# vvvwo/KSS-ICP

Hardware: AMD Instinct MI355X
Metric: icp_iterations_per_sec (higher is better)
Workload: dtype f32; 1 GPU; C2: one 100000x100000 uniform-sphere pair per GPU, 50 fixed ICP iterations + fitness pass per step (exact NN + cov reduce + host 3x3 SVD), R_z(10deg), jitter 1e-3; n_src=100000, n_tgt=100000, pairs_per_gpu=1, nn_engine=cell list + brute-force fallback, nn_arithmetic=reference (no fma)

## Files before the change

### kss-icp_amd/csrc/kss_ctx.hpp

```cpp
#pragma once
#include <dlfcn.h>
#include <hip/hip_runtime.h>

#include <algorithm>
#include <atomic>
#include <chrono>
#include <cmath>
#include <cstdio>
#include <cstdlib>
#include <cstring>
#include <mutex>
#include <string>
#include <thread>
#include <vector>

#include "kss_internal.hpp"
#include "kss_host_pool.hpp"

using namespace kss;

struct DevBuf {
    void* p = nullptr;
    size_t cap = 0;
};

struct kss_ctx {
    int device = 0;
    int cu_count = 0;
    hipStream_t stream = nullptr;
    bool own_stream = false;
    std::string err;
    int nn_mode = KSS_NN_AUTO;
    double grid_stats[8] = {0, 0, 0, 0, 0, 0, 0, 0};
    double last_setup_ms = 0, last_loop_ms = 0;
    double t_launch_us = 0, t_wait_us = 0, t_host_us = 0;
    bool timing = false;
    bool tables_staged = false;
    int64_t stats_ns = -1, stats_nt = -1;

    DevBuf tgt4, src0, cur[2], keys, partials, sums, nn_work, red_work, pair_red, state, cs, scratch_a,
        scratch_b, scratch_c, stage_src, stage_tgt, stage_idx, stage_d2, stage_out, g_counts, g_start, g_cursor,
        g_bsums, g_sorted, g_list, g_count, g_bbox, g_partials, g_start2, g_pairs, g_stamps, g_pos, g_nnst, res_pos, res_wc, res_perm, cand_tags, pack_seg, reg_s, reg_t, reg_p, reg_all, reg_f, reg_g, oct_pts, oct_cen, oct_a, oct_b, oct_tmp, pair_ticket, pre_partials, pre_state, g_rowpair, g_gate;
    HostPool pool;
    std::vector<kss_ctx*> workers;
    std::vector<unsigned long long> last_stamps;
    int stamps_nblk = 0; unsigned long long stamps_seq = 0;
    std::vector<float> h_bbox;
    unsigned int* h_box = nullptr; unsigned int* h_box_dev = nullptr; size_t h_box_bytes = 0;
    unsigned box_tag = 0; int box_rows = 0;
    double evals_sum = 0.0, evals_launches = 0.0;
    void* h_sums = nullptr;  size_t h_sums_cap = 0;
    void* h_sums_dev = nullptr;
    unsigned long long* h_seq = nullptr;
    unsigned long long* h_seq_dev = nullptr;
    size_t h_seq_bytes = 0;
    struct Gated {
        int supported = -1;
        bool want_next = false;
        bool pending = false;
        bool chain = false;
        int steps_left = 0;
        int max_steps = 1;
        int slot = 0;
        unsigned long long seq = 0;
        int32_t stamp = 0;
        const void* d_in = nullptr; void* d_out = nullptr;
        bool fma = false, full = false, want_full = false; double max_d2 = 0.0;
    } gated;
    bool ws_dirty = false;
    bool defer_wait = false;
    PairState* h_xf = nullptr; PairState* h_xf_dev = nullptr;
    bool fit_last = false;
    bool nn_have = false;
    PairState* bar_state = nullptr; int bar_state_cap = 0; bool bar_state_failed = false;
    unsigned int* gate_bar = nullptr;
    unsigned int* res_gate = nullptr; int res_gate_cap = 0; bool res_gate_failed = false;
    unsigned res_launches = 0;
    double res_passes = 0.0;
    int cand_cap = 0, cand_cap_pad = -1, cand_cap_fma = -1;
    int spec_judge = -1; double spec_threshold = 0.0; bool spec_ran = false, spec_cancelled = false;
    std::chrono::steady_clock::time_point res_backoff[2] = {};
    unsigned long long seq = 0;
    void* h_state = nullptr; size_t h_state_cap = 0;

    int prof = 0;
    unsigned prof_tick[KSS_K_COUNT] = {};
    struct EvPair { hipEvent_t a, b; };
    std::vector<EvPair> ev[KSS_K_COUNT];
    std::vector<EvPair> ev_pool;
    double prof_ms[KSS_K_COUNT] = {0};
    int64_t prof_n[KSS_K_COUNT] = {0};
};

static inline int set_err(kss_ctx* c, int code, const char* what, hipError_t e = hipSuccess) {
    if (c) {
        c->err = what;
        if (e != hipSuccess) { c->err += ": "; c->err += hipGetErrorString(e); }
    }
    return code;
}

#define HIPCHK(ctx, call)                                                        \
    do {                                                                         \
        hipError_t e_ = (call);                                                  \
        if (e_ != hipSuccess) return set_err((ctx), KSS_ERR_HIP, #call, e_);     \
    } while (0)

static inline int ensure(kss_ctx* c, DevBuf& b, size_t bytes) {
    if (bytes <= b.cap) return KSS_OK;
    if (b.p) {
        HIPCHK(c, hipStreamSynchronize(c->stream));
        HIPCHK(c, hipFree(b.p));
        b.p = nullptr; b.cap = 0;
    }
    size_t want = bytes + bytes / 8 + 256;
    hipError_t e = hipMalloc(&b.p, want);
    if (e != hipSuccess) { b.p = nullptr; return set_err(c, KSS_ERR_NOMEM, "hipMalloc", e); }
    b.cap = want;
    return KSS_OK;
}

static inline int ensure_zeroed(kss_ctx* c, DevBuf& b, size_t bytes) {
    const size_t before = b.cap;
    const int rc = ensure(c, b, bytes);
    if (rc != KSS_OK) return rc;
    if (b.cap != before && hipMemsetAsync(b.p, 0, b.cap, c->stream) != hipSuccess) return set_err(c, KSS_ERR_HIP, "hipMemsetAsync(zero-at-rest buffer)");
    return KSS_OK;
}

static inline int ensure_pinned(kss_ctx* c, void*& p, size_t& cap, size_t bytes) {
    if (bytes <= cap) return KSS_OK;
    if (p) { HIPCHK(c, hipStreamSynchronize(c->stream)); HIPCHK(c, hipHostFree(p)); p = nullptr; cap = 0; }
    size_t want = bytes * 2 + 256;
    hipError_t e = hipHostMalloc(&p, want, hipHostMallocMapped);
    if (e != hipSuccess) { p = nullptr; return set_err(c, KSS_ERR_NOMEM, "hipHostMalloc", e); }
    cap = want;
    if (&p == &c->h_sums) {
        void* d = nullptr;
        HIPCHK(c, hipHostGetDevicePointer(&d, p, 0));
        c->h_sums_dev = d;
    }
    return KSS_OK;
}

#define KCHK(expr)                     \
    do {                               \
        int rc_ = (expr);              \
        if (rc_ != KSS_OK) return rc_; \
    } while (0)

// ... 54 lines not shown
```

### kss-icp_amd/csrc/kss_engine.hip

```cpp
#pragma clang fp contract(off)

#include <emmintrin.h>

#include "kss_ctx.hpp"

namespace kss {

static int restore_zero_at_rest(kss_ctx* c);
static bool resident_gate_available(kss_ctx* c, int npairs);

static int resident_rows_limit(kss_ctx* c) {
    if (c->cu_count <= 0) {
        hipDeviceProp_t prop;
        c->cu_count = hipGetDeviceProperties(&prop, c->device) == hipSuccess && prop.multiProcessorCount > 0 ? prop.multiProcessorCount : 1;
        (void)hipGetLastError();
    }
    return c->cu_count;
}

constexpr int PUB_PAIRS = 32;
static int ensure_pub(kss_ctx* c, int npairs = PUB_PAIRS);

struct PairGeom {
    int64_t ns, nt;
// ... 469 lines not shown
    }
    return true;
}

static int wait_pair(kss_ctx* c, int p, unsigned long long want) {
    for (long spin = 0; spin < 2000000; ++spin) {
        if (collect_pair(c, p, want)) return KSS_OK;
        __builtin_ia32_pause();
    }
    return KSS_ERR_HIP;
}

static int wait_seq(kss_ctx* c, int npairs = 1, unsigned long long want = 0, const int* active = nullptr, bool* not_published = nullptr) {
    if (!want) want = c->seq;
    bool slow = false;
    for (int p = npairs - 1; p >= 0; --p) {
        if (active && !active[p]) continue;
        if (!slow && wait_pair(c, p, want) == KSS_OK) continue;
        if (!slow) {
            gated_cancel(c);
            HIPCHK(c, hipStreamSynchronize(c->stream));
            slow = true;
        }
        if (!collect_pair(c, p, want)) {
            if (not_published) *not_published = true;
            return set_err(c, KSS_ERR_HIP, "kernel finished without publishing its result");
        }
    }
    return KSS_OK;
}

int ensure_pub_slots(kss_ctx* c) { return ensure_pub(c); }
int wait_slots(kss_ctx* c, int nslots, double* out) {
    const unsigned long long want = c->seq;
    auto collect = [&]() -> bool {
        for (int k = nslots - 1; k >= 0; --k) {
            unsigned long long bits;
            if (!slot_value(c->h_seq, k, want, &bits)) return false;
            std::memcpy(&out[k], &bits, sizeof(double));
        }
        return true;
    };
    for (long spin = 0; spin < 2000000; ++spin) {
        if (collect()) return KSS_OK;
        __builtin_ia32_pause();
    }
    HIPCHK(c, hipStreamSynchronize(c->stream));
    if (!collect()) return set_err(c, KSS_ERR_HIP, "kernel finished without publishing its result");
    return KSS_OK;
}

static bool gated_available(kss_ctx* c) {
    static const bool want = getenv("KSS_GATED") == nullptr || atoi(getenv("KSS_GATED")) != 0;
    if (!want || !c->own_stream || kss_live_contexts().load() != 1) return false;
    if (c->gated.supported < 0) {
        c->gated.supported = 0;
        static const bool want_bar = getenv("KSS_GATE_BAR") == nullptr || atoi(getenv("KSS_GATE_BAR")) != 0;
        hipDeviceProp_t prop;
        void* bar = nullptr;
        if (want_bar && hipGetDeviceProperties(&prop, c->device) == hipSuccess && prop.isLargeBar &&
            hipExtMallocWithFlags(&bar, 4096, hipDeviceMallocFinegrained) == hipSuccess && bar) {
            if (hipMemset(bar, 0, 4096) == hipSuccess && hipDeviceSynchronize() == hipSuccess) {
                c->gate_bar = (unsigned int*)bar;
                c->gated.supported = 1;
                return true;
            }
            hipFree(bar);
        }
        (void)hipGetLastError();
        void *x = nullptr, *xd = nullptr;
        if (ensure(c, c->g_gate, 256) == KSS_OK && hipMemsetAsync(c->g_gate.p, 0, 256, c->stream) == hipSuccess &&
            hipHostMalloc(&x, 2 * sizeof(PairState), hipHostMallocMapped) == hipSuccess && hipHostGetDevicePointer(&xd, x, 0) == hipSuccess) {
            std::memset(x, 0, 2 * sizeof(PairState));
            c->h_xf = (PairState*)x; c->h_xf_dev = (PairState*)xd;
            c->gated.supported = 1;
        } else {
            (void)hipGetLastError();
            if (x) hipHostFree(x);
        }
    }
    return c->gated.supported == 1;
}

static void gated_release(kss_ctx* c, const PairState& st, int skip) {
    if (c->gate_bar) {
        int words[16];
        std::memcpy(words, &st, sizeof st);
        words[14] = skip;
        unsigned int* slot = c->gate_bar + 32 * c->gated.slot;
        static const long torn_at = getenv("KSS_TEST_TORN_GATE") ? atol(getenv("KSS_TEST_TORN_GATE")) : -1;
        static long released = 0;
        const bool torn = ++released == torn_at;
        for (int pass = torn ? 0 : 1; pass < 2; ++pass) {
            for (int g = 0; g < 5; ++g) {
                const unsigned tag = (unsigned)c->gated.stamp + kss_mix3((unsigned)words[3 * g], (unsigned)words[3 * g + 1], (unsigned)words[3 * g + 2]);
                const int w1 = pass == 0 && g == 1 ? words[3 * g + 1] ^ 0x00010000 : words[3 * g + 1];
                const __m128i v = _mm_set_epi32((int)tag, words[3 * g + 2], w1, words[3 * g]);
                _mm_store_si128((__m128i*)(slot + 4 * g), v);
            }
            _mm_sfence();
            if (pass == 0) {
                const auto t0 = std::chrono::steady_clock::now();
                while (std::chrono::duration<double, std::micro>(std::chrono::steady_clock::now() - t0).count() < 200.0) __builtin_ia32_pause();
            }
        }
    } else {
        PairState* rec = &c->h_xf[c->gated.slot];
        for (int k = 0; k < 12; ++k) rec->m[k] = st.m[k];
        rec->active = st.active; rec->apply = st.apply; rec->pad[0] = skip;
        __atomic_store_n(&rec->pad[1], c->gated.stamp, __ATOMIC_RELEASE);
    }
    kss_ctx::Gated& G = c->gated;
    if (!skip && --G.steps_left > 0) {
        G.slot ^= 1;
        G.stamp += 1;
        G.seq += 1;
        const void* in = G.d_out; G.d_out = const_cast<void*>(G.d_in); G.d_in = in;
    } else {
        G.pending = false;
        G.steps_left = 0;
    }
}

static void gated_cancel(kss_ctx* c) {
    if (!c->gated.pending) return;
    PairState none;
    std::memset(&none, 0, sizeof none);
    gated_release(c, none, 1);
}

struct GatedGuard {
    kss_ctx* c;
    explicit GatedGuard(kss_ctx* c_) : c(c_) {}
    ~GatedGuard() { gated_cancel(c); c->gated.want_next = false; }
};

static PassArgs pass_args(kss_ctx* c, const IcpPlan& pl, const float4* d_in, float4* d_out, double max_d2,
                          int32_t* d_idx_out, float* d_d2_out) {
    PassArgs a;
    std::memset(&a, 0, sizeof a);
    a.src_in = d_in; a.src_out = d_out;
    a.cell_start = (const int32_t*)c->g_start.p + 1;
    a.sorted = (const float4*)c->g_sorted.p;
    a.tgt4 = (const float4*)c->tgt4.p;
    a.nn_win = (float4*)c->g_pos.p;
    a.nn_state = (float2*)c->g_nnst.p;
    static const float skin = getenv("KSS_SKIN") ? (float)atof(getenv("KSS_SKIN")) : 0.25f;
    a.skin = skin;
    a.chain_len = 1;
    static const int gate_polls = getenv("KSS_GATE_POLLS") ? atoi(getenv("KSS_GATE_POLLS")) : (1 << 22);
    a.gate_polls = gate_polls;
    a.chained = d_in != (const float4*)c->src0.p ? 1 : c->fit_last ? 2 : 0;
    a.src_last0 = (const float4*)c->cur[0].p; a.src_last1 = (const float4*)c->cur[1].p;
    a.keys = (unsigned long long*)c->keys.p;
    a.list = (int32_t*)c->g_list.p; a.list_count = (int32_t*)c->g_count.p;
    a.total_rows = pl.total_rows;
    static const bool noprev = getenv("KSS_GRID_NOPREV") != nullptr;
    a.use_prev = !noprev && c->nn_have ? 1 : 0;
    a.max_d2 = max_d2;
    a.rows = (double*)c->partials.p; a.tickets = (int32_t*)c->pair_ticket.p;
    a.pub = c->h_seq_dev;
    a.idx_out = d_idx_out; a.d2_out = d_d2_out;
    {
        static const long torn_at = getenv("KSS_TEST_TORN_SLOT") ? atol(getenv("KSS_TEST_TORN_SLOT")) : -1;
        static long launches = 0;
        a.test_torn = torn_at > 0 && ++launches == torn_at ? 1 : 0;
    }
    if (pl.gridb) {
        a.pairs = (const GridPairDev*)c->g_pairs.p;
        a.row_pair = (const int32_t*)c->g_rowpair.p;
    } else {
        a.pair0 = pl.gpairs[0];
        static const bool tagged = getenv("KSS_TAGGED_ROWS") == nullptr || atoi(getenv("KSS_TAGGED_ROWS")) != 0;
        static const int tagged_max = getenv("KSS_TAGGED_ROWS_MAX") ? atoi(getenv("KSS_TAGGED_ROWS_MAX")) : (1 << 30);
        a.tagged_rows = tagged && pl.total_rows <= std::max(tagged_max, resident_rows_limit(c)) ? 1 : 0;
    }
    return a;
}

static int nn_pass(kss_ctx* c, const IcpPlan& pl, bool fma, const float4* d_in, float4* d_out, double max_d2,
            int32_t* d_idx_out, float* d_d2_out, bool full, const int* active = nullptr) {
    PairState* hs = (PairState*)c->h_state;
    if (pl.grid) {
        PassArgs a = pass_args(c, pl, d_in, d_out, max_d2, d_idx_out, d_d2_out);
        const int nblk = grid_pass_blocks(pl.total_rows);
        static const int stamps_mode = getenv("KSS_GRID_STAMPS") ? atoi(getenv("KSS_GRID_STAMPS")) : 0;
        unsigned long long* stamps2 = nullptr;
        if (stamps_mode == 1) {
            KCHK(ensure(c, c->g_stamps, (size_t)nblk * 16 * sizeof(unsigned long long)));
            HIPCHK(c, hipMemsetAsync(c->g_stamps.p, 0, (size_t)nblk * 16 * sizeof(unsigned long long), c->stream));
            a.stamps = (unsigned long long*)c->g_stamps.p;
        } else if (stamps_mode == 2) {
            KCHK(ensure(c, c->g_stamps, (size_t)nblk * 32 * sizeof(unsigned long long)));
            stamps2 = (unsigned long long*)c->g_stamps.p;
            c->stamps_nblk = nblk;
        }
        const auto tl0 = c->timing ? std::chrono::steady_clock::now() : std::chrono::steady_clock::time_point();
        unsigned long long want_seq = 0;
        bool via_gate = false;
        kss_ctx::Gated& G = c->gated;
        const bool plain_args = !a.stamps && !d_idx_out && !d_d2_out;
        if (G.pending && G.d_in == (const void*)d_in && G.d_out == (void*)d_out && G.fma == fma && G.full == full && G.max_d2 == max_d2 && plain_args) {
            want_seq = G.seq;
            c->seq = std::max(c->seq, G.seq);
            if (G.chain && c->prof > 0) c->prof_n[KSS_K_GRID_CHAIN_PASS] += 1;
            via_gate = true;
            static const long drop_at = getenv("KSS_TEST_DROP_GATE") ? atol(getenv("KSS_TEST_DROP_GATE")) : -1;
            static long releases = 0;
            if (++releases == drop_at) { G.pending = false; G.steps_left = 0; }
            else gated_release(c, hs[0], 0);
        } else {
            gated_cancel(c);
            ProfScope ps(c, KSS_K_GRID_NN);
            a.ps0 = hs[0];
            a.seq = ++c->seq;
            if (stamps2) a.stamps = stamps2 + (size_t)(a.seq & 1) * nblk * 16;
            launch_grid_pass(c->stream, fma, full, false, true, a);
            c->nn_have = true;
            want_seq = c->seq;
        }
        HIPCHK(c, hipGetLastError());
        const bool next_sampled = c->prof == 1 || (c->prof > 1 && c->prof_tick[KSS_K_GRID_NN] % (unsigned)c->prof == 0);
        static const bool want_chain = getenv("KSS_CHAIN") == nullptr || atoi(getenv("KSS_CHAIN")) != 0;
        int len = 1;
        if (G.want_next && !G.pending && plain_args && gated_available(c) && want_chain && c->gate_bar &&
            ((a.tagged_rows && pl.total_rows <= resident_rows_limit(c)) || pl.total_rows == 1))
            len = std::max(1, std::min(G.max_steps, 1 << 16));
        if (G.want_next && !G.pending && plain_args && gated_available(c) && (len > 1 || !next_sampled)) {
            if (c->prof > 1 && len == 1) ++c->prof_tick[KSS_K_GRID_NN];
            float4* nxt_out = d_out == (float4*)c->cur[0].p ? (float4*)c->cur[1].p : (float4*)c->cur[0].p;
            G.slot ^= 1;
            G.stamp = (G.stamp + 1) & 0x7fffffff;
            if (G.stamp == 0 || G.stamp > 0x7fffffff - len - 1) G.stamp = 1;
            PassArgs n = pass_args(c, pl, d_out, nxt_out, max_d2, nullptr, nullptr);
            n.ps0 = hs[0];
            n.gate_seq = G.stamp;
            if (c->gate_bar) {
                n.state = nullptr;
                n.gate_dev = c->gate_bar;
                n.gate_slot = G.slot;
                n.chain_len = len;
                n.src_alt = d_out;
            } else {
                n.state = c->h_xf_dev + G.slot;
                n.gate_dev = (unsigned int*)c->g_gate.p;
            }
            n.seq = c->seq + 1;
            if (stamps2) n.stamps = stamps2 + (size_t)(n.seq & 1) * nblk * 16;
            if (len > 1) {
                ProfScope ps(c, KSS_K_GRID_CHAIN, true);
                launch_grid_pass(c->stream, fma, G.want_full, false, true, n);
            } else {
                launch_grid_pass(c->stream, fma, G.want_full, false, true, n);
            }
            G.chain = len > 1;
            G.pending = true; G.steps_left = len; G.seq = n.seq; G.d_in = d_out; G.d_out = nxt_out; G.fma = fma; G.full = G.want_full; G.max_d2 = max_d2;
            if (hipGetLastError() != hipSuccess) { gated_cancel(c); G.supported = 0; }
        }
        const auto tl1 = c->timing ? std::chrono::steady_clock::now() : std::chrono::steady_clock::time_point();
        {
            bool not_published = false;
            int rcw = wait_seq(c, 1, want_seq, nullptr, &not_published);
            if (rcw != KSS_OK && via_gate && not_published) {
                G.pending = false; G.steps_left = 0;
                c->err.clear();
                std::fprintf(stderr, "[kss] a waiting kernel was not answered in time and left; the pass is launched again\n");
                c->ws_dirty = true;
                KCHK(restore_zero_at_rest(c));
                ProfScope ps(c, KSS_K_GRID_NN);
                a.ps0 = hs[0];
                a.seq = ++c->seq;
                launch_grid_pass(c->stream, fma, full, false, true, a);
                HIPCHK(c, hipGetLastError());
                want_seq = c->seq;
                rcw = wait_seq(c, 1, want_seq);
            }
            KCHK(rcw);
        }
        if (stamps2) c->stamps_seq = want_seq;
        if (c->timing) {
            const auto tl2 = std::chrono::steady_clock::now();
            c->t_launch_us += std::chrono::duration<double, std::micro>(tl1 - tl0).count();
            c->t_wait_us += std::chrono::duration<double, std::micro>(tl2 - tl1).count();
        }
        if (a.stamps && !stamps2) {
            c->last_stamps.resize((size_t)nblk * 16);
            HIPCHK(c, hipMemcpy(c->last_stamps.data(), a.stamps, c->last_stamps.size() * sizeof(unsigned long long), hipMemcpyDeviceToHost));
            for (int b = 0; b < nblk; ++b) c->evals_sum += (double)c->last_stamps[(size_t)b * 16 + 10];
            c->evals_launches += 1.0;
        }
        if (((const double*)c->h_sums)[NSUMS - 1] > 0.0) {
            gated_cancel(c);
            c->gated.want_next = false;
            KCHK(stage_tables(c, pl));
            {
                PairState one;
                std::memset(&one, 0, sizeof one);
                one.active = 1;
                HIPCHK(c, hipMemcpy(c->state.p, &one, sizeof one, hipMemcpyHostToDevice));
            }
            if (getenv("KSS_LIST_CHECK")) {
                HIPCHK(c, hipStreamSynchronize(c->stream));
                int32_t cnt = -1;
                HIPCHK(c, hipMemcpy(&cnt, c->g_count.p, sizeof cnt, hipMemcpyDeviceToHost));
                const int64_t ns0 = pl.g[0].ns;
                std::vector<int32_t> l((size_t)std::max<int64_t>(0, std::min<int64_t>(cnt, ns0)));
                if (!l.empty()) HIPCHK(c, hipMemcpy(l.data(), c->g_list.p, l.size() * sizeof(int32_t), hipMemcpyDeviceToHost));
                int64_t bad = 0;
                for (int32_t v : l) bad += v < 0 || v >= ns0;
                std::fprintf(stderr, "[kss] list check: count %d of %lld sources (column 19 said %.0f), %lld entries out of range, nn table %zu items, S %d\n",
                             cnt, (long long)ns0, ((const double*)c->h_sums)[NSUMS - 1], (long long)bad, pl.nn.size(), pl.S);
                if (cnt < 0 || cnt > ns0 || bad) return set_err(c, KSS_ERR_HIP, "list check failed");
            }
            {
                ProfScope ps(c, KSS_K_NN_SWEEP);
                launch_nn_sweep_list(c->stream, pl.S, fma, (const NNWork*)c->nn_work.p, (int)pl.nn.size(), (const PairState*)c->state.p,
                                     d_out, (const float4*)c->tgt4.p, (unsigned long long*)c->keys.p, (const int32_t*)c->g_list.p,
                                     (const int32_t*)c->g_count.p);
            }
            HIPCHK(c, hipMemsetAsync(c->g_count.p, 0, sizeof(int32_t), c->stream));
            {
                ProfScope ps(c, KSS_K_CORR_REDUCE);
                PassArgs r = pass_args(c, pl, d_in, d_out, max_d2, d_idx_out, d_d2_out);
                r.ps0 = hs[0];
                r.seq = ++c->seq;
                launch_grid_pass(c->stream, fma, true, false, false, r);
            }
            HIPCHK(c, hipGetLastError());
            KCHK(wait_seq(c, 1, c->seq));
        }
        ((double*)c->h_sums)[NSUMS - 1] = 0.0;
        return KSS_OK;
    }
    if (pl.gridb) {
        PassArgs a = pass_args(c, pl, d_in, d_out, max_d2, d_idx_out, d_d2_out);
        a.state = (const PairState*)c->state.p;
        if (c->bar_state && c->bar_state_cap >= pl.npairs) {
            _mm_sfence();
            a.state = c->bar_state;
        }
        static const int host_state_rows = [] { const char* e = getenv("KSS_BATCH_HOST_STATE_ROWS"); return e ? atoi(e) : 32768; }();
        if (a.state != c->bar_state && pl.total_rows <= host_state_rows) {
            void* dev = nullptr;
            if (hipHostGetDevicePointer(&dev, c->h_state, 0) == hipSuccess && dev) a.state = (const PairState*)dev;
        }
        if (a.state == (const PairState*)c->state.p)
            HIPCHK(c, hipMemcpyAsync(c->state.p, hs, (size_t)pl.npairs * sizeof(PairState), hipMemcpyHostToDevice, c->stream));
// ... 566 lines not shown
    }
    const double max_d2 = P.max_corr_dist * P.max_corr_dist;
    const double* hsum = (const double*)c->h_sums;
    if (P.trace_n) *P.trace_n = 0;
    int n_active = P.max_iterations > 0 ? np : 0;
    if (P.max_iterations <= 0)
        for (int p = 0; p < np; ++p) { active[p] = 0; }
    int it = 0;
    GatedGuard gated_guard(c);

    auto solve_pairs = [&](int p0, int p1, unsigned long long pass_seq, bool poll_first, int* n_finished) -> int {
        std::atomic<int> finished{0}, stuck{0};
        bool poll = poll_first;
        std::fill(solved.begin() + p0, solved.begin() + p1, 0);
        auto solve = [&](int pb, int pe) {
            int fin_here = 0;
            for (int p = pb; p < pe; ++p) {
                if (!active[p] || solved[p]) continue;
                if (poll && wait_pair(c, p, pass_seq) != KSS_OK) { stuck.fetch_add(1); continue; }
                const double* s = hsum + (size_t)p * NSUMS;
                if ((int)s[0] < P.min_correspondences) {
                    state[p] = KSS_STATE_NO_CORRESPONDENCES; converged[p] = 0; active[p] = 0; ++fin_here; solved[p] = 1;
                    set_state(hs[p], I, 0, 0);
                    mirror_state(bar, p, hs[p]);
                    continue;
                }
                float* tk = &Tk[(size_t)p * 16];
                rigid_from_sums(s, tk);
                mat4_mul(tk, &fin[(size_t)p * 16], &fin[(size_t)p * 16]);
                ++iters[p];
                const double mse = s[16] / s[0];
                last_mse[p] = mse;
                if (p == 0 && P.trace_n && *P.trace_n < P.trace_cap) {
                    if (P.trace_sums) std::memcpy(P.trace_sums + (size_t)(*P.trace_n) * NSUMS, s, NSUMS * sizeof(double));
                    if (P.trace_Tk) std::memcpy(P.trace_Tk + (size_t)(*P.trace_n) * 16, tk, 16 * sizeof(float));
                    ++*P.trace_n;
                }
                const bool done = conv[p].has_converged(iters[p], tk, mse);
                state[p] = conv[p].state;
                solved[p] = 1;
                if (done) {
                    converged[p] = 1; active[p] = 0; ++fin_here;
                    set_state(hs[p], tk, 0, 1);
                } else {
                    set_state(hs[p], tk, 1, 1);
                }
                mirror_state(bar, p, hs[p]);
            }
            finished.fetch_add(fin_here, std::memory_order_relaxed);
        };
        const int n = p1 - p0;
        if (n >= 64) {
            std::atomic<int> next{0};
            static const int kBlock = [] { const char* e = getenv("KSS_SOLVE_BLOCK"); const int v = e ? atoi(e) : 0; return v > 0 ? v : 64; }();
            c->pool.parallel_for(n, [&](int, int) {
                for (;;) {
                    const int pb = p0 + next.fetch_add(1) * kBlock;
                    if (pb >= p1) break;
                    solve(pb, std::min(p1, pb + kBlock));
                }
            });
        } else {
            solve(p0, p1);
        }
        if (stuck.load() > 0) {
            HIPCHK(c, hipStreamSynchronize(c->stream));
            for (int p = p0; p < p1; ++p) {
                if (!active[p] || solved[p]) continue;
                if (!collect_pair(c, p, pass_seq)) return set_err(c, KSS_ERR_HIP, "kernel finished without publishing its result");
            }
            poll = false;
            solve(p0, p1);
        }
        *n_finished = finished.load(std::memory_order_relaxed);
        return KSS_OK;
    };

    while (n_active > 0) {
        const float4* d_in = it == 0 ? (const float4*)c->src0.p : (const float4*)c->cur[(it - 1) & 1].p;
        float4* d_out = (float4*)c->cur[it & 1].p;
        c->gated.want_next = plan->grid && !P.allreduce && it + 1 < P.max_iterations;
        c->gated.want_full = full;
        c->gated.max_steps = P.max_iterations - (it + 1);
        c->defer_wait = plan->gridb;
        const auto tb0 = c->timing ? std::chrono::steady_clock::now() : std::chrono::steady_clock::time_point();
        const int rc_pass = nn_pass(c, *plan, P.nn_fma != 0, d_in, d_out, max_d2, nullptr, nullptr, full, active.data());
        const bool deferred = c->defer_wait;
        c->defer_wait = false;
        const auto tb1 = c->timing ? std::chrono::steady_clock::now() : std::chrono::steady_clock::time_point();
        KCHK(rc_pass);
        const unsigned long long pass_seq = c->seq;
        if (P.allreduce && P.allreduce(P.allreduce_user, (double*)c->h_sums, NSUMS) != 0)
            return set_err(c, KSS_ERR_RCCL, "icp: the allreduce callback failed");
        if (plan->gridb) was_active = active;
        int fin_now = 0;
        KCHK(solve_pairs(0, np, pass_seq, deferred, &fin_now));
        if (c->timing && deferred) {
            const auto tb2 = std::chrono::steady_clock::now();
            c->t_launch_us += std::chrono::duration<double, std::micro>(tb1 - tb0).count();
            c->t_wait_us += std::chrono::duration<double, std::micro>(tb2 - tb1).count();
        }
        if (plan->gridb) {
            double fallback = 0.0, act = 0.0;
            for (int p = 0; p < np; ++p)
                if (was_active[p]) { fallback += hsum[(size_t)p * NSUMS + NSUMS - 1]; act += (double)plan->g[p].ns; }
            if (fallback > 0.10 * act && !getenv("KSS_GRID_NOSWITCH")) {
                std::vector<int64_t> ns(np), nt(np);
                for (int p = 0; p < np; ++p) { ns[p] = plan->g[p].ns; nt[p] = plan->g[p].nt; }
                KCHK(build_plan(c, ns.data(), nt.data(), np, pl_in.shared_target, P.nn_sources_per_thread, P.nn_target_splits, KSS_NN_BRUTE, brute_plan));
                brute_plan.src_in_cell_order = true;
                KCHK(stage_plan(c, brute_plan));
                plan = &brute_plan;
            }
        }
        n_active -= fin_now;
        ++it;
    }
    for (int p = 0; p < np; ++p) {
        kss_icp_result& r = results[p];
        std::memcpy(r.T, &fin[(size_t)p * 16], 16 * sizeof(float));
        r.iterations = iters[p]; r.converged = converged[p]; r.state = state[p];
        r.last_mse = last_mse[p]; r.fitness = 0.0; r.pair_id = p;
    }
    if (P.compute_fitness) {
        const bool cell_lists = plan->grid || plan->gridb;
        for (int p = 0; p < np; ++p) {
            set_state(hs[p], &fin[(size_t)p * 16], 1, 1);
            if (cell_lists && plan == &pl_in && iters[p] >= 1 && state[p] != KSS_STATE_NO_CORRESPONDENCES) hs[p].pad[0] = 1 + ((iters[p] - 1) & 1);
            mirror_state(bar, p, hs[p]);
        }
        c->fit_last = cell_lists && plan == &pl_in;
        struct FitGuard { kss_ctx* c; ~FitGuard() { c->fit_last = false; } } fit_guard{c};
        c->gated.want_next = false;
        int32_t* d_idx = nullptr;
        float* d_d2 = nullptr;
        if (P.fitness_idx || P.fitness_d2) {
            KCHK(ensure(c, c->stage_idx, (size_t)plan->total_src * sizeof(int32_t)));
            KCHK(ensure(c, c->stage_d2, (size_t)plan->total_src * sizeof(float)));
            d_idx = (int32_t*)c->stage_idx.p; d_d2 = (float*)c->stage_d2.p;
        }
        KCHK(nn_pass(c, *plan, P.nn_fma != 0, (const float4*)c->src0.p, (float4*)c->cur[0].p, max_d2, d_idx, d_d2, true));
        if (P.allreduce) {
            double v[2] = {hsum[17], (double)plan->g[0].ns};
            if (P.allreduce(P.allreduce_user, v, 2) != 0) return set_err(c, KSS_ERR_RCCL, "icp: the allreduce callback failed");
            results[0].fitness = v[0] / v[1];
        } else {
            for (int p = 0; p < np; ++p) results[p].fitness = hsum[(size_t)p * NSUMS + 17] / (double)plan->g[p].ns;
        }
        if (d_idx) {
            const size_t n0 = (size_t)plan->g[0].ns;
            if (P.fitness_idx) HIPCHK(c, hipMemcpyAsync(P.fitness_idx, d_idx, n0 * sizeof(int32_t), hipMemcpyDeviceToHost, c->stream));
            if (P.fitness_d2) HIPCHK(c, hipMemcpyAsync(P.fitness_d2, d_d2, n0 * sizeof(float), hipMemcpyDeviceToHost, c->stream));
            HIPCHK(c, hipStreamSynchronize(c->stream));
        }
    }
    return KSS_OK;
}

static int restore_zero_at_rest(kss_ctx* c) {
    if (!c->ws_dirty) return KSS_OK;
    HIPCHK(c, hipStreamSynchronize(c->stream));
    for (DevBuf* b : {&c->pair_ticket, &c->g_count, &c->g_counts})
        if (b->p) HIPCHK(c, hipMemsetAsync(b->p, 0, b->cap, c->stream));
    c->ws_dirty = false;
    return KSS_OK;
}
// ... 79 lines not shown
```

### kss-icp_amd/csrc/kss_grid.hip

```cpp
#pragma clang fp contract(off)

#include <hip/hip_runtime.h>

#include <cstring>

#include <rocprim/rocprim.hpp>

#include <cstdlib>

#include "kss_internal.hpp"
#include "kss_device.hpp"

namespace kss {

__global__ __launch_bounds__(256) void grid_count2_kernel(const float4* __restrict__ tgt, int nt, int nbt, const float4* __restrict__ src, int ns,
                                                          GridParams gp, int32_t* __restrict__ counts) {
    const bool is_src = (int)blockIdx.x >= nbt;
    const int i = ((int)blockIdx.x - (is_src ? nbt : 0)) * 256 + (int)threadIdx.x;
    if (i >= (is_src ? ns : nt)) return;
    const float4 p = is_src ? src[i] : tgt[i];
    const int cx = cell_coord(p.x, gp.ox, gp.inv_h, gp.gx), cy = cell_coord(p.y, gp.oy, gp.inv_h, gp.gy),
              cz = cell_coord(p.z, gp.oz, gp.inv_h, gp.gz);
    atomicAdd(&counts[(is_src ? gp.gx * gp.gy * gp.gz : 0) + (cz * gp.gy + cy) * gp.gx + cx], 1);
}
// ... 493 lines not shown
                const int ls = atomicAdd(a.list_count, 1);
                a.list[ls] = io;
                wfell = true;
            }
            a.nn_win[io] = make_float4(ww.x, ww.y, ww.z, __uint_as_float(whave ? (unsigned)wkey : ~0u));
            a.nn_state[io] = make_float2(wfell ? 0.f : bnew, 0.f);
            s_ent[WK_X][owner] = __float_as_uint(ww.x); s_ent[WK_Y][owner] = __float_as_uint(ww.y); s_ent[WK_Z][owner] = __float_as_uint(ww.z);
            s_ent[WK_IDX][owner] = (unsigned)wkey; s_ent[WK_D2][owner] = (unsigned)(wkey >> 32);
            s_ent[WK_FL][owner] = (whave ? 1u : 0u) | (wfell ? 2u : 0u);
            s_ent[WK_R][owner] = __float_as_uint(wfell ? 0.f : bnew);
        }
        KSS_STAMP(8);
        if (a.stamps) {
            int evs = evl, mx = evl;
#pragma unroll
            for (int m = 32; m > 0; m >>= 1) { evs += __shfl_xor(evs, m, 64); mx = max(mx, __shfl_xor(mx, m, 64)); }
            if (lane == 0) {
                atomicAdd(&a.stamps[(size_t)blockIdx.x * 16 + 10], (unsigned long long)evs);
                atomicAdd(&a.stamps[(size_t)blockIdx.x * 16 + 11], (unsigned long long)(((mx + 7) / 8) * 8 * 64));
            }
        }
    }
#undef KSS_STAMP
}

#ifndef KSS_BATCH_WAVES
#define KSS_BATCH_WAVES 6
#endif
#ifndef KSS_SINGLE_WAVES
#define KSS_SINGLE_WAVES 1
#endif
template <bool FMA, bool FULL, bool BATCH, bool SEARCH, bool CHAIN>
__global__ __launch_bounds__(PASS_BS, BATCH ? KSS_BATCH_WAVES : KSS_SINGLE_WAVES) void grid_pass_kernel(const PassArgs a) {
    static_assert(!CHAIN || (!BATCH && SEARCH), "chained launches: single pair, search passes");
#define KSS_STAMP(k) do { if (a.stamps && threadIdx.x == 0) a.stamps[(size_t)blockIdx.x * 16 + (k)] = __builtin_amdgcn_s_memrealtime(); } while (0)
    KSS_STAMP(0);
    constexpr int BS = PASS_BS;
    const int per_xcd = (int)gridDim.x / 8;
    const int w = ((int)blockIdx.x % 8) * per_xcd + (int)blockIdx.x / 8;
    if (w >= a.total_rows) return;
    int pi = 0;
    if constexpr (BATCH) pi = a.row_pair[w];
    const GridPairDev pr = BATCH ? a.pairs[pi] : a.pair0;
    PairState ps = a.ps0;
    if constexpr (BATCH) {
        ps = a.state[pi];
        if (!ps.active) return;
    }
    const GridParams& gp = pr.gp;
    const int32_t* __restrict__ cs = a.cell_start + pr.cell_base;
    const float4* __restrict__ sorted = a.sorted;
    constexpr int WQ = 256;
    __shared__ int2 rowq[9][WQ];
    __shared__ double shw[BS / 64][NSUMS];
    __shared__ int s_last;
    __shared__ int sh_ps[16];
    __shared__ int s_nwalk;
    __shared__ unsigned s_ent[7][BS];
    __shared__ unsigned short s_wl[BS];
    enum { WK_X, WK_Y, WK_Z, WK_IDX, WK_D2, WK_R, WK_POS, WK_FL = WK_POS, WK_COLS };
    static_assert(sizeof(PairState) == 64, "the gated launch reads the transform record as 16 dwords");
    double (*shf)[NSUMS] = reinterpret_cast<double (*)[NSUMS]>(&rowq[0][0]);
    static_assert(sizeof(double) * PASS_FG * NSUMS <= sizeof(int2) * 9 * WQ, "shf must fit inside rowq");

    const int local = (w - pr.row_base) * BS + (int)threadIdx.x;
    const bool valid = local < pr.src_n;
    const int i = pr.src_base + local;
    const int lane = threadIdx.x & 63, wave = threadIdx.x >> 6;
    bool have = false, fell_back = false;
    float qx = 0.f, qy = 0.f, qz = 0.f, d2 = 0.f;
    float4 win = make_float4(0.f, 0.f, 0.f, 0.f);
    float4 p = make_float4(0.f, 0.f, 0.f, 0.f), prevp = make_float4(0.f, 0.f, 0.f, __uint_as_float(~0u));
    float2 st = make_float2(0.f, 0.f);
    if (valid) {
        p = SEARCH ? a.src_in[i] : a.src_out[i];
        if (!SEARCH || a.use_prev) { prevp = a.nn_win[i]; st = a.nn_state[i]; }
    }
    for (int step = 0;; ++step) {
    const bool last_step = !CHAIN || step + 1 >= a.chain_len;
    const unsigned long long seq_k = a.seq + (unsigned long long)step;
    const int gate_k = a.gate_seq != 0 ? a.gate_seq + step : 0;
    unsigned int* const gate_ptr = a.gate_dev + 32 * ((a.gate_slot + step) & 1);
    float4* const src_out_k = (step & 1) ? a.src_alt : a.src_out;
    const bool last_known = a.chained == 2 && ps.pad[0] > 0;
    const bool chained_k = step > 0 || a.chained == 1 || last_known;
    const bool has_prev = __float_as_uint(prevp.w) != ~0u;
    if constexpr (SEARCH) {
        __syncthreads();
        if (threadIdx.x == 0) s_nwalk = 0;
        __syncthreads();
    }
    KSS_STAMP(13);
    if constexpr (!BATCH && SEARCH) {
        if (gate_k != 0) {
            typedef unsigned int u32x4 __attribute__((ext_vector_type(4)));
            if (a.state && w == 0 && threadIdx.x < 16) {
                const int* w32 = reinterpret_cast<const int*>(a.state);
                int v = 0, n = 0;
                bool ok = true;
                for (;;) {
                    v = __hip_atomic_load(w32 + threadIdx.x, __ATOMIC_RELAXED, __HIP_MEMORY_SCOPE_SYSTEM);
                    if (__shfl(v, 15, 64) == gate_k) break;
                    __builtin_amdgcn_s_sleep(1);
                    if (++n > a.gate_polls / 2) { ok = false; break; }
                }
                if (ok) {
                    const int g = threadIdx.x;
                    const int w0 = __shfl(v, min(3 * g, 15), 64), w1 = __shfl(v, min(3 * g + 1, 15), 64), w2 = __shfl(v, min(3 * g + 2, 15), 64);
                    if (g < 5) {
                        u32x4 o;
                        o.x = (unsigned)w0; o.y = (unsigned)w1; o.z = (unsigned)w2; o.w = (unsigned)gate_k + kss_mix3(o.x, o.y, o.z);
                        unsigned int* dst = gate_ptr + 4 * g;
                        asm volatile("global_store_dwordx4 %0, %1, off sc1" ::"v"(dst), "v"(o) : "memory");
                    }
                }
            }
            if (threadIdx.x < 8) {
                const unsigned int* src = gate_ptr + 4 * min((int)threadIdx.x, 4);
                u32x4 v;
                int n = 0;
                bool ok = true;
                for (;;) {
                    asm volatile("global_load_dwordx4 %0, %1, off sc0 sc1\n\ts_waitcnt vmcnt(0)" : "=&v"(v) : "v"(src) : "memory");
                    if (__builtin_amdgcn_ballot_w64(v.w - kss_mix3(v.x, v.y, v.z) == (unsigned)gate_k) == 0xffull) break;
                    __builtin_amdgcn_s_sleep(1);
                    if (++n > a.gate_polls) { ok = false; break; }
                }
                if (threadIdx.x < 5) { sh_ps[3 * threadIdx.x] = (int)v.x; sh_ps[3 * threadIdx.x + 1] = (int)v.y; sh_ps[3 * threadIdx.x + 2] = (int)v.z; }
                if (threadIdx.x == 0) { sh_ps[15] = gate_k; s_last = ok ? 1 : 0; }
            }
            __syncthreads();
            if (!s_last) return;
            int* d32 = reinterpret_cast<int*>(&ps);
#pragma unroll
            for (int k = 0; k < 16; ++k) d32[k] = sh_ps[k];
            if (ps.pad[0] != 0) return;
            __syncthreads();
            KSS_STAMP(9);
        }
    }
    unsigned long long key = ~0ull;
    float pold_x = p.x, pold_y = p.y, pold_z = p.z;
    if (SEARCH && last_known && valid) {
        const float4 pl = (ps.pad[0] == 1 ? a.src_last0 : a.src_last1)[i];
        pold_x = pl.x; pold_y = pl.y; pold_z = pl.z;
    }
    if (valid) {
        if constexpr (SEARCH) {
            if (ps.apply) {
                const float x = p.x, y = p.y, z = p.z;
                p.x = ((ps.m[0] * x + ps.m[1] * y) + ps.m[2] * z) + ps.m[3];
                p.y = ((ps.m[4] * x + ps.m[5] * y) + ps.m[6] * z) + ps.m[7];
                p.z = ((ps.m[8] * x + ps.m[9] * y) + ps.m[10] * z) + ps.m[11];
            }
            src_out_k[i] = p;
        }
        qx = p.x; qy = p.y; qz = p.z;
        const bool qok = (qx - qx) == 0.f && (qy - qy) == 0.f && (qz - qz) == 0.f;
        if constexpr (!SEARCH) {
            if (has_prev) {
                win = prevp;
                key = point_key<FMA>(win, qx, qy, qz);
            } else if (qok) {
                key = a.keys[i];
                if (key != ~0ull) win = a.tgt4[pr.tgt_base + (int)(unsigned)(key & 0xffffffffull)];
            }
            have = key != ~0ull;
        }
    }
    if constexpr (SEARCH) {
        bool walker = false;
        float acc_keep = 0.f;
        {
            const bool qok = valid && (qx - qx) == 0.f && (qy - qy) == 0.f && (qz - qz) == 0.f;
            const SkipOut so = skip_test<FMA>(qok, qx, qy, qz, pold_x, pold_y, pold_z, prevp, st, chained_k, a.skin, gp.h);
            walker = so.walker;
            key = so.key;
            acc_keep = so.acc;
            unsigned fl = 0u;
            if (qok && !walker) {
                fl = 1u;
                a.nn_state[i] = make_float2(st.x, so.acc);
            } else if (valid && !qok) {
                a.nn_win[i] = make_float4(0.f, 0.f, 0.f, __uint_as_float(~0u));
                a.nn_state[i] = make_float2(0.f, 0.f);
            }
            const float4 c4 = walker ? make_float4(qx, qy, qz, 0.f) : prevp;
            s_ent[WK_X][threadIdx.x] = __float_as_uint(c4.x); s_ent[WK_Y][threadIdx.x] = __float_as_uint(c4.y); s_ent[WK_Z][threadIdx.x] = __float_as_uint(c4.z);
            s_ent[WK_IDX][threadIdx.x] = (unsigned)key; s_ent[WK_D2][threadIdx.x] = (unsigned)(key >> 32);
            s_ent[WK_POS][threadIdx.x] = walker ? (unsigned)so.kpos : fl;
            s_ent[WK_R][threadIdx.x] = __float_as_uint(so.rho);
        }
        const unsigned long long wm = __builtin_amdgcn_ballot_w64(walker);
        if (wm != 0ull) {
            int base = 0;
            if (lane == 0) base = atomicAdd(&s_nwalk, (int)__builtin_popcountll(wm));
            base = __builtin_amdgcn_readfirstlane(base);
            if (walker) s_wl[base + (int)__builtin_amdgcn_mbcnt_hi((unsigned)(wm >> 32), __builtin_amdgcn_mbcnt_lo((unsigned)wm, 0u))] = (unsigned short)threadIdx.x;
        }
        KSS_STAMP(14);
        __syncthreads();
        const int nwalk = s_nwalk;
        if (a.stamps && threadIdx.x == 0) a.stamps[(size_t)blockIdx.x * 16 + 12] = (unsigned long long)nwalk;
        serve_walkers<FMA, BATCH, WQ, BS, BATCH ? 4 : 8>(a, pr, cs, sorted, w, nwalk, rowq, s_ent, s_wl);
        KSS_STAMP(15);
        __syncthreads();
        {
            const unsigned fl = s_ent[WK_FL][threadIdx.x];
            have = (fl & 1u) != 0u; fell_back = (fl & 2u) != 0u;
            win = make_float4(__uint_as_float(s_ent[WK_X][threadIdx.x]), __uint_as_float(s_ent[WK_Y][threadIdx.x]), __uint_as_float(s_ent[WK_Z][threadIdx.x]), 0.f);
            key = ((unsigned long long)s_ent[WK_D2][threadIdx.x] << 32) | (unsigned long long)s_ent[WK_IDX][threadIdx.x];
            if (CHAIN && !last_step) {
                if (walker) {
                    prevp = make_float4(win.x, win.y, win.z, __uint_as_float(have ? (unsigned)key : ~0u));
                    st = make_float2(__uint_as_float(s_ent[WK_R][threadIdx.x]), 0.f);
                } else if (have) {
                    st.y = acc_keep;
                } else {
                    prevp.w = __uint_as_float(~0u);
                    st = make_float2(0.f, 0.f);
                }
            }
        }
// ... 651 lines not shown
```

Baseline: 79980 iterations/s.

## Pre-launch gated fitness pass alongside ICP chain to hide launch latency

Measured after the change: 80560 iterations/s, median of 6. No clear change (+0.7%).

```diff
diff --git a/kss-icp_amd/csrc/kss_ctx.hpp b/kss-icp_amd/csrc/kss_ctx.hpp
--- a/kss-icp_amd/csrc/kss_ctx.hpp
+++ b/kss-icp_amd/csrc/kss_ctx.hpp
@@ -66,6 +66,10 @@
         int32_t stamp = 0;
         const void* d_in = nullptr; void* d_out = nullptr;
         bool fma = false, full = false, want_full = false; double max_d2 = 0.0;
+        bool want_fit = false;
+        bool fit_pending = false;
+        int32_t fit_stamp = 0;
+        unsigned long long fit_seq = 0;
     } gated;
     bool ws_dirty = false;
     bool defer_wait = false;
diff --git a/kss-icp_amd/csrc/kss_engine.hip b/kss-icp_amd/csrc/kss_engine.hip
--- a/kss-icp_amd/csrc/kss_engine.hip
+++ b/kss-icp_amd/csrc/kss_engine.hip
@@ -575,32 +575,35 @@
     return c->gated.supported == 1;
 }
 
+static void gate_write_bar(unsigned int* slot, int32_t stamp, const PairState& st, int skip) {
+    int words[16];
+    std::memcpy(words, &st, sizeof st);
+    words[14] = skip ? -1 : st.pad[0];
+    static const long torn_at = getenv("KSS_TEST_TORN_GATE") ? atol(getenv("KSS_TEST_TORN_GATE")) : -1;
+    static long released = 0;
+    const bool torn = ++released == torn_at;
+    for (int pass = torn ? 0 : 1; pass < 2; ++pass) {
+        for (int g = 0; g < 5; ++g) {
+            const unsigned tag = (unsigned)stamp + kss_mix3((unsigned)words[3 * g], (unsigned)words[3 * g + 1], (unsigned)words[3 * g + 2]);
+            const int w1 = pass == 0 && g == 1 ? words[3 * g + 1] ^ 0x00010000 : words[3 * g + 1];
+            const __m128i v = _mm_set_epi32((int)tag, words[3 * g + 2], w1, words[3 * g]);
+            _mm_store_si128((__m128i*)(slot + 4 * g), v);
+        }
+        _mm_sfence();
+        if (pass == 0) {
+            const auto t0 = std::chrono::steady_clock::now();
+            while (std::chrono::duration<double, std::micro>(std::chrono::steady_clock::now() - t0).count() < 200.0) __builtin_ia32_pause();
+        }
+    }
+}
+
 static void gated_release(kss_ctx* c, const PairState& st, int skip) {
     if (c->gate_bar) {
-        int words[16];
-        std::memcpy(words, &st, sizeof st);
-        words[14] = skip;
-        unsigned int* slot = c->gate_bar + 32 * c->gated.slot;
-        static const long torn_at = getenv("KSS_TEST_TORN_GATE") ? atol(getenv("KSS_TEST_TORN_GATE")) : -1;
-        static long released = 0;
-        const bool torn = ++released == torn_at;
-        for (int pass = torn ? 0 : 1; pass < 2; ++pass) {
-            for (int g = 0; g < 5; ++g) {
-                const unsigned tag = (unsigned)c->gated.stamp + kss_mix3((unsigned)words[3 * g], (unsigned)words[3 * g + 1], (unsigned)words[3 * g + 2]);
-                const int w1 = pass == 0 && g == 1 ? words[3 * g + 1] ^ 0x00010000 : words[3 * g + 1];
-                const __m128i v = _mm_set_epi32((int)tag, words[3 * g + 2], w1, words[3 * g]);
-                _mm_store_si128((__m128i*)(slot + 4 * g), v);
-            }
-            _mm_sfence();
-            if (pass == 0) {
-                const auto t0 = std::chrono::steady_clock::now();
-                while (std::chrono::duration<double, std::micro>(std::chrono::steady_clock::now() - t0).count() < 200.0) __builtin_ia32_pause();
-            }
-        }
+        gate_write_bar(c->gate_bar + 32 * c->gated.slot, c->gated.stamp, st, skip);
     } else {
         PairState* rec = &c->h_xf[c->gated.slot];
         for (int k = 0; k < 12; ++k) rec->m[k] = st.m[k];
-        rec->active = st.active; rec->apply = st.apply; rec->pad[0] = skip;
+        rec->active = st.active; rec->apply = st.apply; rec->pad[0] = skip ? -1 : st.pad[0];
         __atomic_store_n(&rec->pad[1], c->gated.stamp, __ATOMIC_RELEASE);
     }
     kss_ctx::Gated& G = c->gated;
@@ -615,17 +618,33 @@
     }
 }
 
-static void gated_cancel(kss_ctx* c) {
+static unsigned int* fit_record(kss_ctx* c) { return c->gate_bar + 64; }
+
+static void fit_release(kss_ctx* c, const PairState& st, int skip) {
+    gate_write_bar(fit_record(c), c->gated.fit_stamp, st, skip);
+    c->gated.fit_pending = false;
+}
+
+static void gated_cancel_chain(kss_ctx* c) {
     if (!c->gated.pending) return;
     PairState none;
     std::memset(&none, 0, sizeof none);
     gated_release(c, none, 1);
 }
 
+static void gated_cancel(kss_ctx* c) {
+    gated_cancel_chain(c);
+    if (c->gated.fit_pending) {
+        PairState none;
+        std::memset(&none, 0, sizeof none);
+        fit_release(c, none, 1);
+    }
+}
+
 struct GatedGuard {
     kss_ctx* c;
     explicit GatedGuard(kss_ctx* c_) : c(c_) {}
-    ~GatedGuard() { gated_cancel(c); c->gated.want_next = false; }
+    ~GatedGuard() { gated_cancel(c); c->gated.want_next = false; c->gated.want_fit = false; }
 };
 
 static PassArgs pass_args(kss_ctx* c, const IcpPlan& pl, const float4* d_in, float4* d_out, double max_d2,
@@ -693,15 +712,27 @@
         bool via_gate = false;
         kss_ctx::Gated& G = c->gated;
         const bool plain_args = !a.stamps && !d_idx_out && !d_d2_out;
-        if (G.pending && G.d_in == (const void*)d_in && G.d_out == (void*)d_out && G.fma == fma && G.full == full && G.max_d2 == max_d2 && plain_args) {
-            want_seq = G.seq;
-            c->seq = std::max(c->seq, G.seq);
-            if (G.chain && c->prof > 0) c->prof_n[KSS_K_GRID_CHAIN_PASS] += 1;
+        const bool next_waits = G.pending && G.d_in == (const void*)d_in && G.d_out == (void*)d_out && G.fma == fma && G.full == full &&
+                                G.max_d2 == max_d2 && plain_args;
+        const bool fit_waits = !next_waits && G.fit_pending && c->fit_last && d_in == (const float4*)c->src0.p && d_out == (float4*)c->cur[0].p &&
+                               full && G.fma == fma && G.max_d2 == max_d2 && plain_args;
+        if (next_waits || fit_waits) {
+            if (fit_waits) gated_cancel_chain(c);
+            const unsigned long long s = fit_waits ? G.fit_seq : G.seq;
+            want_seq = s;
+            c->seq = std::max(c->seq, s);
+            if (next_waits && G.chain && c->prof > 0) c->prof_n[KSS_K_GRID_CHAIN_PASS] += 1;
             via_gate = true;
             static const long drop_at = getenv("KSS_TEST_DROP_GATE") ? atol(getenv("KSS_TEST_DROP_GATE")) : -1;
             static long releases = 0;
-            if (++releases == drop_at) { G.pending = false; G.steps_left = 0; }
-            else gated_release(c, hs[0], 0);
+            if (++releases == drop_at) {
+                if (fit_waits) G.fit_pending = false;
+                else { G.pending = false; G.steps_left = 0; }
+            } else if (fit_waits) {
+                fit_release(c, hs[0], 0);
+            } else {
+                gated_release(c, hs[0], 0);
+            }
         } else {
             gated_cancel(c);
             ProfScope ps(c, KSS_K_GRID_NN);
@@ -748,6 +779,19 @@
             }
             G.chain = len > 1;
             G.pending = true; G.steps_left = len; G.seq = n.seq; G.d_in = d_out; G.d_out = nxt_out; G.fma = fma; G.full = G.want_full; G.max_d2 = max_d2;
+            if (len > 1 && G.want_fit && c->prof == 0 && !stamps2) {
+                PassArgs f = pass_args(c, pl, (const float4*)c->src0.p, (float4*)c->cur[0].p, max_d2, nullptr, nullptr);
+                f.chained = 2;
+                f.ps0 = hs[0];
+                G.fit_stamp = (G.fit_stamp + 1) & 0x7fffffff;
+                if (G.fit_stamp == 0) G.fit_stamp = 1;
+                f.gate_seq = G.fit_stamp;
+                f.gate_dev = fit_record(c);
+                f.gate_slot = 0;
+                f.seq = n.seq + (unsigned long long)len;
+                launch_grid_pass(c->stream, fma, true, false, true, f);
+                G.fit_pending = true; G.fit_seq = f.seq;
+            }
             if (hipGetLastError() != hipSuccess) { gated_cancel(c); G.supported = 0; }
         }
         const auto tl1 = c->timing ? std::chrono::steady_clock::now() : std::chrono::steady_clock::time_point();
@@ -755,7 +799,7 @@
             bool not_published = false;
             int rcw = wait_seq(c, 1, want_seq, nullptr, &not_published);
             if (rcw != KSS_OK && via_gate && not_published) {
-                G.pending = false; G.steps_left = 0;
+                G.pending = false; G.steps_left = 0; G.fit_pending = false;
                 c->err.clear();
                 std::fprintf(stderr, "[kss] a waiting kernel was not answered in time and left; the pass is launched again\n");
                 c->ws_dirty = true;
@@ -1488,6 +1532,7 @@
         c->gated.want_next = plan->grid && !P.allreduce && it + 1 < P.max_iterations;
         c->gated.want_full = full;
         c->gated.max_steps = P.max_iterations - (it + 1);
+        c->gated.want_fit = plan->grid && P.compute_fitness && !P.fitness_idx && !P.fitness_d2;
         c->defer_wait = plan->gridb;
         const auto tb0 = c->timing ? std::chrono::steady_clock::now() : std::chrono::steady_clock::time_point();
         const int rc_pass = nn_pass(c, *plan, P.nn_fma != 0, d_in, d_out, max_d2, nullptr, nullptr, full, active.data());
diff --git a/kss-icp_amd/csrc/kss_grid.hip b/kss-icp_amd/csrc/kss_grid.hip
--- a/kss-icp_amd/csrc/kss_grid.hip
+++ b/kss-icp_amd/csrc/kss_grid.hip
@@ -599,8 +599,6 @@
     const int gate_k = a.gate_seq != 0 ? a.gate_seq + step : 0;
     unsigned int* const gate_ptr = a.gate_dev + 32 * ((a.gate_slot + step) & 1);
     float4* const src_out_k = (step & 1) ? a.src_alt : a.src_out;
-    const bool last_known = a.chained == 2 && ps.pad[0] > 0;
-    const bool chained_k = step > 0 || a.chained == 1 || last_known;
     const bool has_prev = __float_as_uint(prevp.w) != ~0u;
     if constexpr (SEARCH) {
         __syncthreads();
@@ -651,11 +649,13 @@
             int* d32 = reinterpret_cast<int*>(&ps);
 #pragma unroll
             for (int k = 0; k < 16; ++k) d32[k] = sh_ps[k];
-            if (ps.pad[0] != 0) return;
+            if (ps.pad[0] < 0) return;
             __syncthreads();
             KSS_STAMP(9);
         }
     }
+    const bool last_known = a.chained == 2 && ps.pad[0] > 0;
+    const bool chained_k = step > 0 || a.chained == 1 || last_known;
     unsigned long long key = ~0ull;
     float pold_x = p.x, pold_y = p.y, pold_z = p.z;
     if (SEARCH && last_known && valid) {
```
